# codex-storage/codex-storage-proofs-circuits

Measured on AMD Instinct MI355X. Metric: Poseidon2-BN254 permutations/sec per GPU; full proof-input witnesses/sec, higher is better.
Workload: dtype u32x9 (29-bit limbs, Montgomery mod BN254 r)

## Files before the change

### codex-storage-proofs-circuits_amd/csrc/internal.hpp

```cpp
#pragma once
#include <hip/hip_runtime.h>

#include <sys/resource.h>
#include <sys/syscall.h>
#include <unistd.h>

#include <condition_variable>
#include <cstdint>
#include <deque>
#include <functional>
#include <memory>
#include <mutex>
#include <string>
#include <thread>
#include <vector>

#include "../../include/codex_p2.h"
#include "workers.hpp"

namespace cp2i {

bool env_decimal(const char* name, uint64_t* value, bool* set);
bool env_keep_trees(int* mode);
size_t mem_limit_bytes();
hipError_t dev_malloc(void** p, size_t n);
void dev_free(void* p, size_t n);
size_t dev_bytes_held();
int device_free_bytes(size_t* out);

class BlockPool {
 public:
  static constexpr size_t MAX_CACHED_DEV = (size_t)6 << 30, MAX_CACHED_PIN = (size_t)4 << 30;
  ~BlockPool() { trim(); }
  void* get(bool pinned, size_t n, size_t* got) {
    if (n == 0) n = 16;
    {
      std::lock_guard<std::mutex> lk(mu_);
      auto& fl = pinned ? pin_ : dev_;
      size_t best = fl.size();
      for (size_t i = 0; i < fl.size(); ++i)
        if (fl[i].bytes >= n && fl[i].bytes / 4 <= n && (best == fl.size() || fl[i].bytes < fl[best].bytes)) best = i;
      if (best != fl.size()) {
        Blk b = fl[best];
        fl.erase(fl.begin() + (long)best);
        (pinned ? cached_pin_ : cached_dev_) -= b.bytes;
        *got = b.bytes;
        return b.p;
      }
    }
    size_t want = round_up(n);
    void* p = nullptr;
    hipError_t e = pinned ? hipHostMalloc(&p, want, hipHostMallocDefault) : dev_malloc(&p, want);
    if (e != hipSuccess) {
      (void)hipGetLastError();
      trim();
// ... 235 lines not shown
```

### codex-storage-proofs-circuits_amd/csrc/proof_many.cpp

```cpp
#include <hip/hip_runtime.h>

#include <algorithm>
#include <cstring>
#include <map>
#include <memory>
#include <string>
#include <vector>

#include "dataset_obj.hpp"
#include "proof_input_obj.hpp"
#include "trees.hpp"

using namespace cp2i;

namespace {

struct Req {
  cp2_dataset* ds = nullptr;
  uint64_t slot = 0;
  uint8_t entropy[32];
  size_t at = 0;
  size_t id = 0;
};

int refuse(cp2_ctx* ctx, size_t i, const std::string& why) {
  ctx->err = "request " + std::to_string(i) + ": " + why;
  return CP2_ERR_INVALID;
}

size_t depth_of(size_t n) { return layer_sizes_of(n).size() - 1; }

bool same_circuit(const cp2_config& a, const cp2_config& b) {
  return a.max_depth == b.max_depth && a.max_log2_nslots == b.max_log2_nslots && a.cell_size == b.cell_size && a.block_size == b.block_size &&
// ... 31 lines not shown
  CP2_TRY(d_a.scratch(ctx, n * 8));
  CP2_TRY(d_r.scratch(ctx, n * 32));
  CP2_HIP(ctx, hipMemcpyAsync(d_a.p, a.data(), n * 8, hipMemcpyHostToDevice, ctx->stream));
  CP2_HIP(ctx, cp2k::launch_gather_addr(static_cast<const uint64_t*>(d_a.p), n, 32, d_r.p, ctx->stream));
  CP2_HIP(ctx, hipMemcpyAsync(got.data(), d_r.p, n * 32, hipMemcpyDeviceToHost, ctx->stream));
  CP2_HIP(ctx, hipStreamSynchronize(ctx->stream));
  for (size_t i = 0; i < n; ++i)
    if (std::memcmp(&got[i * 32], &ds[i]->dlayers[slot_idx[i] * 32], 32) != 0)
      return refuse(ctx, i, "the root its dataset tree holds for slot " + std::to_string(slot_idx[i]) +
                                " (cp2_dataset_set_roots) differs from the slot's built root");
  return CP2_OK;
}

int prepare(cp2_ctx* ctx, cp2_dataset* const* ds, const uint64_t* slot_idx, size_t n) {
  CP2_TRY(validate(ctx, ds, slot_idx, n));
  CP2_HIP(ctx, hipSetDevice(ctx->device));
  for (size_t i = 0; i < n; ++i)
    if (!ds[i]->have_roots) CP2_TRY(cp2_dataset_set_roots(ds[i], nullptr));
  return check_roots(ctx, ds, slot_idx, n);
}

std::string who(bool named, const Req* r) { return named ? "request " + std::to_string(r->id) + ": " : std::string(); }

int run_pass(cp2_ctx* ctx, const std::vector<const Req*>& rq, size_t n_rf, size_t n_rfile, size_t n_cf, bool named, cp2_proof_input** out) {
  const size_t n = rq.size(), nr = n_rf + n_rfile;
  const cp2_config& c0 = rq[0]->ds->cfg;
  const size_t ns = c0.n_samples, md = (size_t)c0.max_depth, cs = c0.cell_size, bs = c0.block_size, cpb = bs / cs;
  const size_t T = n * ns, R = nr * ns, C = T - R, RF = n_rf * ns, CF = n_cf * ns;
  auto store = std::make_shared<BatchStore>();
  if (T) {
    std::vector<cp2k::ManyReq> reqs(n);
    std::vector<cp2k::TreeGeom> geoms;
    std::map<std::string, uint32_t> geom_of;
    for (size_t j = 0; j < n; ++j) {
      const cp2_dataset* ds = rq[j]->ds;
      cp2k::ManyReq& q = reqs[j];
      std::memset(&q, 0, sizeof q);
      std::memcpy(q.entropy, rq[j]->entropy, 32);
      std::memcpy(q.slot_root, &ds->dlayers[rq[j]->slot * 32], 32);
      q.n_cells = ds->cfg.n_cells;
      q.cpb = cpb;
      if (j < nr) {
        cp2k::TreeGeom g;
        std::memset(&g, 0, sizeof g);
        trees_geom(ds->trees, &g);
        auto it = geom_of.emplace(std::string(reinterpret_cast<const char*>(&g), sizeof g), (uint32_t)geoms.size());
        if (it.second) geoms.push_back(g);
        q.geom = it.first->second;
        q.nodes = (uint64_t)reinterpret_cast<uintptr_t>(ds->trees->nodes.p);
        q.slot = rq[j]->slot - ds->first_slot;
      }
    }
    std::vector<uint64_t> blk(C), gen, cpaths, ctail, ccell;
    std::vector<uint8_t> checks(2 * C * 32);
    PinBuf h_blocks;
    const size_t rows = T * md + T + 2 * C;
    DevBuf d_req, d_geom, d_idx, d_blk, d_addr, d_rows, d_cells, d_gen, d_caddr;
    CP2_TRY(d_req.scratch(ctx, n * sizeof(cp2k::ManyReq)));
    CP2_TRY(d_geom.scratch(ctx, std::max<size_t>(1, geoms.size()) * sizeof(cp2k::TreeGeom)));
    CP2_TRY(d_idx.scratch(ctx, T * 8));
    CP2_TRY(d_blk.scratch(ctx, T * 8));
    CP2_TRY(d_addr.scratch(ctx, rows * 8));
    CP2_TRY(d_rows.scratch(ctx, rows * 32));
    CP2_TRY(d_cells.scratch(ctx, (C * cpb + T) * cs));
    CP2_TRY(store->idx.alloc(ctx, T * 8));
    CP2_TRY(store->paths.alloc(ctx, T * md * 32));
    CP2_TRY(store->leaves.alloc(ctx, T * 32));
    CP2_TRY(store->cells.alloc(ctx, T * cs));
    uint8_t* cells_out = d_cells.u8() + C * cpb * cs;
    uint64_t* addr = static_cast<uint64_t*>(d_addr.p);
    CP2_HIP(ctx, hipMemcpyAsync(d_req.p, reqs.data(), n * sizeof(cp2k::ManyReq), hipMemcpyHostToDevice, ctx->stream));
    if (!geoms.empty())
      CP2_HIP(ctx, hipMemcpyAsync(d_geom.p, geoms.data(), geoms.size() * sizeof(cp2k::TreeGeom), hipMemcpyHostToDevice, ctx->stream));
    CP2_HIP(ctx, cp2k::launch_sample_many(static_cast<const cp2k::ManyReq*>(d_req.p), static_cast<const cp2k::TreeGeom*>(d_geom.p), n,
                                          (uint32_t)ns, (uint32_t)md, static_cast<uint64_t*>(d_idx.p), static_cast<uint64_t*>(d_blk.p), addr,
                                          ctx->stream));
    CP2_HIP(ctx, hipMemcpyAsync(store->idx.p, d_idx.p, T * 8, hipMemcpyDeviceToHost, ctx->stream));
    if (C) CP2_HIP(ctx, hipMemcpyAsync(blk.data(), static_cast<uint64_t*>(d_blk.p) + R, C * 8, hipMemcpyDeviceToHost, ctx->stream));
    CP2_HIP(ctx, hipStreamSynchronize(ctx->stream));
    const uint64_t* idx = static_cast<const uint64_t*>(store->idx.p);

    gen.assign((CF + RF) * 2, 0);
    uint64_t* seeds = gen.data();
    uint64_t* firsts = seeds + CF + RF;
    for (size_t q = 0; q < CF; ++q) {
      const Req* r = rq[nr + q / ns];
      seeds[q] = cp2_slot_seed(r->ds->cfg.seed, r->slot);
      firsts[q] = blk[q] * cpb;
    }
    for (size_t p = 0; p < RF; ++p) {
      const Req* r = rq[p / ns];
      seeds[CF + p] = cp2_slot_seed(r->ds->cfg.seed, r->slot);
      firsts[CF + p] = idx[p];
    }
    if (CF + RF) {
      CP2_TRY(d_gen.scratch(ctx, gen.size() * 8));
      const uint64_t* dg = static_cast<const uint64_t*>(d_gen.p);
      CP2_HIP(ctx, hipMemcpyAsync(d_gen.p, gen.data(), gen.size() * 8, hipMemcpyHostToDevice, ctx->stream));
      CP2_HIP(ctx, cp2k::launch_gen_fake_cells_many(dg, dg + CF + RF, cpb, CF * cpb, cs, d_cells.p, ctx->stream));
      CP2_HIP(ctx, cp2k::launch_gen_fake_cells_many(dg + CF, dg + CF + RF + CF, 1, RF, cs, cells_out, ctx->stream));
    }
    if (C > CF) {
      const size_t n_req_file = (C - CF) / ns;
      CP2_TRY(h_blocks.alloc(ctx, (C - CF) * bs));
      std::vector<std::string> failed(fill_threads(ctx));
      on_threads(fill_threads(ctx), n_req_file, [&](int w, size_t k) {
        const size_t q0 = CF + k * ns;
        const Req* r = rq[nr + q0 / ns];
        const std::string fname = slot_file_name(r->ds->file_base, r->slot);
        size_t bad = 0;
        const int err = slot_file_read_list(fname, ns, [&](size_t) { return bs; }, [&](size_t c) { return blk[q0 + c] * bs; },
                                            [&](size_t c) { return h_blocks.u8() + (q0 - CF + c) * bs; }, &bad);
        if (err >= 0)
          failed[w] = who(named, r) + (err ? "block " + std::to_string(blk[q0 + bad]) + " of slot " : std::string("slot ")) + std::to_string(r->slot) +
                      ": " + slot_file_error(fname, err);
        return err < 0;
      });
      for (const auto& f : failed)
        if (!f.empty()) { ctx->err = f; return CP2_ERR_IO; }
      CP2_HIP(ctx, hipMemcpyAsync(d_cells.u8() + CF * bs, h_blocks.p, (C - CF) * bs, hipMemcpyHostToDevice, ctx->stream));
    }
    cp2_slot_trees* mini = nullptr;
    struct Mini { cp2_slot_trees*& t; ~Mini() { cp2_slot_trees_free(t); } } mini_guard{mini};
    if (C) {
      cpaths.assign(C * md, 0);
      ctail.assign(3 * C, 0);
      ccell.assign(C, 0);
      CP2_TRY(cp2_slot_trees_build_dev(ctx, d_cells.p, C, cs, bs, cpb, &mini));
      const size_t depth_b = depth_of(cpb);
      const uint64_t mb = (uint64_t)reinterpret_cast<uintptr_t>(mini->nodes.p);
      std::vector<uint64_t> rr(depth_b + 1);
      for (size_t q = 0; q < C; ++q) {
        const Req* r = rq[nr + q / ns];
        const cp2_dataset* ds = r->ds;
        const uint64_t ls = r->slot - ds->first_slot, cell = idx[R + q], b = blk[q], in_block = cell % cpb;
        const uint64_t kb = (uint64_t)reinterpret_cast<uintptr_t>(ds->compact.p);
        uint64_t* P = &cpaths[q * md];
        path_rows(mini, q, in_block, depth_b + 1, rr.data());
        for (size_t d = 0; d < depth_b; ++d) P[d] = rr[d] == NO_ROW ? 0 : mb + rr[d] * 32;
        uint64_t j = b, m = ds->cfg.n_cells / cpb;
        for (size_t d = 0; d + 1 < ds->csizes.size(); ++d) {
          const uint64_t sib = j ^ 1;
          P[depth_b + d] = sib < m ? kb + (ds->coff[d] + ls * ds->csizes[d] + sib) * 32 : 0;
          j >>= 1;
          m = (m + 1) >> 1;
        }
        ctail[q] = mb + (q * cpb + in_block) * 32;
        ctail[C + 2 * q] = kb + (ds->coff[0] + ls * ds->csizes[0] + b) * 32;
        ctail[C + 2 * q + 1] = mb + (mini->toff[0] + q) * 32;
        ccell[q] = (uint64_t)reinterpret_cast<uintptr_t>(d_cells.u8()) + (q * cpb + in_block) * cs;
      }
      CP2_TRY(d_caddr.scratch(ctx, C * 8));
      CP2_HIP(ctx, hipMemcpyAsync(addr + R * md, cpaths.data(), C * md * 8, hipMemcpyHostToDevice, ctx->stream));
      CP2_HIP(ctx, hipMemcpyAsync(addr + T * md + R, ctail.data(), 3 * C * 8, hipMemcpyHostToDevice, ctx->stream));
      CP2_HIP(ctx, hipMemcpyAsync(d_caddr.p, ccell.data(), C * 8, hipMemcpyHostToDevice, ctx->stream));
      CP2_HIP(ctx, cp2k::launch_gather_addr(static_cast<const uint64_t*>(d_caddr.p), C, cs, cells_out + R * cs, ctx->stream));
    }
    CP2_HIP(ctx, cp2k::launch_gather_addr(addr, rows, 32, d_rows.p, ctx->stream));
    CP2_HIP(ctx, hipMemcpyAsync(store->paths.p, d_rows.p, T * md * 32, hipMemcpyDeviceToHost, ctx->stream));
    CP2_HIP(ctx, hipMemcpyAsync(store->leaves.p, d_rows.u8() + T * md * 32, T * 32, hipMemcpyDeviceToHost, ctx->stream));
    if (C) CP2_HIP(ctx, hipMemcpyAsync(checks.data(), d_rows.u8() + (T * md + T) * 32, 2 * C * 32, hipMemcpyDeviceToHost, ctx->stream));
    CP2_HIP(ctx, hipMemcpyAsync(store->cells.p, cells_out, T * cs, hipMemcpyDeviceToHost, ctx->stream));
    CP2_HIP(ctx, hipStreamSynchronize(ctx->stream));
    for (size_t q = 0; q < C; ++q)
      if (std::memcmp(&checks[2 * q * 32], &checks[(2 * q + 1) * 32], 32) != 0) {
        const Req* r = rq[nr + q / ns];
        ctx->err = who(named, r) + "block " + std::to_string(blk[q]) + " of slot " + std::to_string(r->slot) +
                   " does not hash to its stored root (slot data changed since the build?)";
        return CP2_ERR_IO;
      }
    if (R > RF) {
      std::vector<std::string> failed(fill_threads(ctx));
      on_threads(fill_threads(ctx), n_rfile, [&](int w, size_t k) {
        const Req* r = rq[n_rf + k];
        const std::string fname = slot_file_name(r->ds->file_base, r->slot);
        const size_t p0 = (n_rf + k) * ns;
        const int err = slot_file_read_list(fname, ns, [&](size_t) { return cs; }, [&](size_t c) { return idx[p0 + c] * cs; },
                                            [&](size_t c) { return store->cells.u8() + (p0 + c) * cs; });
        if (err >= 0) failed[w] = who(named, r) + slot_file_error(fname, err);
        return err < 0;
      });
      for (const auto& f : failed)
        if (!f.empty()) { ctx->err = f; return CP2_ERR_IO; }
    }
  }
  std::vector<ProofItem> items(n);
  for (size_t j = 0; j < n; ++j) items[j] = {rq[j]->ds, rq[j]->slot, rq[j]->entropy, &out[rq[j]->at]};
  return proof_inputs_from_store(items.data(), n, store, store->cells.u8());
}

}

int cp2i::prove_requests(cp2_ctx* ctx, cp2_dataset* const* ds, const uint64_t* slot_idx, const uint8_t* entropies, size_t n, size_t at0,
                         bool named, cp2_proof_input** out) {
  for (size_t i = 0; i < n; ++i) out[i] = nullptr;
  if (n == 0) return CP2_OK;
  CP2_HIP(ctx, hipSetDevice(ctx->device));
  std::vector<Req> req(n);
  std::vector<const Req*> res_fake, res_file, cmp_fake, cmp_file, roots_only;
  for (size_t i = 0; i < n; ++i) {
    req[i].ds = ds[i];
    req[i].slot = slot_idx[i];
    req[i].at = i;
    req[i].id = at0 + i;
    canonical_felt(entropies + 32 * i, req[i].entropy);
    const cp2_dataset* d = ds[i];
    (d->trees ? (d->from_file ? res_file : res_fake) : d->tree_mode == 2 ? (d->from_file ? cmp_file : cmp_fake) : roots_only).push_back(&req[i]);
  }
  auto fail = [&](int st) {
    for (size_t i = 0; i < n; ++i) { cp2_proof_input_free(out[i]); out[i] = nullptr; }
    return st;
  };
  for (const Req* r : roots_only) {
    const int st = cp2_proof_inputs_generate_batch(r->ds, &r->slot, 1, r->entropy, &out[r->at]);
    if (st != CP2_OK) {
      ctx->err = who(named, r) + ctx->err;
      return fail(st);
    }
  }
  const cp2_config& c0 = ds[0]->cfg;
  const size_t per_req = std::max<size_t>(1, (size_t)c0.n_samples * c0.block_size);
  const size_t chunk = std::max<size_t>(1, ctx->stage_bytes / per_req);
  std::vector<const Req*> compact(cmp_fake);
  compact.insert(compact.end(), cmp_file.begin(), cmp_file.end());
  const size_t n_res = res_fake.size() + res_file.size();
  size_t c = 0;
  for (bool first = true; first ? n_res + compact.size() > 0 : c < compact.size(); first = false) {
    std::vector<const Req*> rq;
    if (first) {
      rq = res_fake;
      rq.insert(rq.end(), res_file.begin(), res_file.end());
    }
    const size_t c1 = std::min(compact.size(), c + chunk);
    rq.insert(rq.end(), compact.begin() + (long)c, compact.begin() + (long)c1);
    const size_t n_cf = c < cmp_fake.size() ? std::min(c1, cmp_fake.size()) - c : 0;
    const int st = run_pass(ctx, rq, first ? res_fake.size() : 0, first ? res_file.size() : 0, n_cf, named, out);
    if (st != CP2_OK) return fail(st);
    c = c1;
  }
  return CP2_OK;
}

extern "C" int cp2_proof_inputs_generate_many(cp2_ctx* ctx, cp2_dataset* const* ds, const uint64_t* slot_idx, const uint8_t* entropies, size_t n,
                                              cp2_proof_input** out) try {
  if (!ctx) return CP2_ERR_INVALID;
  if (n && (!ds || !slot_idx || !entropies || !out)) {
    ctx->err = "cp2_proof_inputs_generate_many: NULL array";
    return CP2_ERR_INVALID;
  }
  for (size_t i = 0; i < n; ++i) out[i] = nullptr;
  if (n == 0) return CP2_OK;
  CP2_REFUSE_STUCK(ctx);
  CP2_TRY(prepare(ctx, ds, slot_idx, n));
  return prove_requests(ctx, ds, slot_idx, entropies, n, 0, true, out);
} catch (const std::bad_alloc&) {
  return CP2_ERR_ALLOC;
} catch (...) {
  return CP2_ERR_INVALID;
}

extern "C" int cp2_proof_inputs_export_many(cp2_ctx* ctx, cp2_dataset* const* ds, const uint64_t* slot_idx, const uint8_t* entropies, size_t n,
                                            const char* const* paths, int threads, size_t batch, uint64_t* total_bytes) try {
  if (!ctx) return CP2_ERR_INVALID;
// ... 17 lines not shown
```

### codex-storage-proofs-circuits_amd/csrc/slot_trees.cpp

```cpp
#include <hip/hip_runtime.h>

#include <fcntl.h>
#include <sys/mman.h>
#include <sys/stat.h>
#include <unistd.h>

#include <algorithm>
#include <atomic>
#include <chrono>
#include <cstdio>
#include <cstdlib>
#include <cstring>
#include <memory>
#include <new>
#include <string>
#include <vector>

#include "trees.hpp"
#include "fake_turns.hpp"
#include "ingest_turns.hpp"
#include "fill_pipeline.hpp"

using namespace cp2i;

// ... 270 lines not shown
  if (!ctx || !out || units_per_slot == 0) return CP2_ERR_INVALID;
  CP2_TRY(trees_check_geometry(cell_size, block_size, cells_per_unit, n_units));
  if (units_per_slot > 1 && !unit_geometry_ok(units_per_slot, cell_size, block_size, cells_per_unit)) return CP2_ERR_INVALID;
  return trees_build_fake(ctx, dataset_seed, first_unit, n_units, cell_size, block_size, cells_per_unit, 0, nullptr, out, units_per_slot);
} catch (const std::bad_alloc&) {
  return CP2_ERR_ALLOC;
} catch (...) {
  return CP2_ERR_INVALID;
}

extern "C" int cp2_slot_trees_build_file_units(cp2_ctx* ctx, const char* file_base, uint64_t units_per_slot, uint64_t first_unit,
                                               size_t n_units, size_t cell_size, size_t block_size, size_t cells_per_unit,
                                               cp2_slot_trees** out) try {
  if (!ctx || !out || !file_base || units_per_slot == 0 || cell_size > SLOT_FILE_MAX_CELL) return CP2_ERR_INVALID;
  CP2_TRY(trees_check_geometry(cell_size, block_size, cells_per_unit, n_units));
  if (units_per_slot > 1 && !unit_geometry_ok(units_per_slot, cell_size, block_size, cells_per_unit)) return CP2_ERR_INVALID;
  return trees_build_files(ctx, file_base, first_unit, n_units, cell_size, block_size, cells_per_unit, 0, nullptr, out, units_per_slot);
} catch (const std::bad_alloc&) {
  return CP2_ERR_ALLOC;
} catch (...) {
  return CP2_ERR_INVALID;
}

extern "C" int cp2_slot_trees_build_dev(cp2_ctx* ctx, const void* d_cells, size_t n_slots, size_t cell_size,
                                        size_t block_size, size_t n_cells, cp2_slot_trees** out) try {
  if (!ctx || !out || !d_cells) return CP2_ERR_INVALID;
  *out = nullptr;
  CP2_REFUSE_STUCK(ctx);
  CP2_TRY(trees_check_geometry(cell_size, block_size, n_cells, n_slots));
  CP2_HIP(ctx, hipSetDevice(ctx->device));
  std::unique_ptr<cp2_slot_trees> t(trees_new(ctx, n_slots, cell_size, block_size, n_cells));
  if (!t) return CP2_ERR_ALLOC;
  t->src = CellSrc::Dev;
  t->d_cells = static_cast<const uint8_t*>(d_cells);
  CP2_TRY(trees_layout(t.get()));
  CP2_HIP(ctx, cp2k::launch_hash_cells(d_cells, cell_size, n_slots * n_cells, t->nodes.p, ctx->stream));
  CP2_TRY(trees_build_layers(t.get(), 0, n_slots, ctx->stream));
  *out = t.release();
  return CP2_OK;
} catch (const std::bad_alloc&) {
  return CP2_ERR_ALLOC;
} catch (...) {
  return CP2_ERR_INVALID;
}

namespace {

size_t env_size(const char* name, size_t dflt) {
  const char* v = std::getenv(name);
  if (!v || !*v) return dflt;
  char* end = nullptr;
  unsigned long long x = std::strtoull(v, &end, 10);
  return (end && *end == 0 && x > 0) ? (size_t)x : dflt;
}

struct IngestPipe {
  static constexpr int MAX_DEPTH = 8;
  static constexpr size_t DIRECT_ALIGN = 4096;
  size_t cell_multiple = 1;
  cp2_ctx* ctx = nullptr;
  hipStream_t copy = nullptr;
  int pin_depth = 0, dev_depth = 0;
// ... 618 lines not shown
```

### codex-storage-proofs-circuits_amd/csrc/trees.hpp

```cpp
#pragma once
#include <functional>
#include <string>
#include <vector>

#include "batch_loop.hpp"
#include "internal.hpp"
#include "kernels.hpp"
#include "fill_pipeline.hpp"
#include "cache_file.hpp"

struct cp2_slot_trees {
  cp2_ctx* ctx = nullptr;
  size_t n_slots = 0, cell_size = 0, block_size = 0, n_cells = 0, cpb = 0, nblocks = 0;
  std::vector<size_t> bsizes, tsizes;
  std::vector<size_t> boff, toff;
  cp2i::DevBuf nodes;
  CellSrc src = CellSrc::Fake;
  uint64_t dataset_seed = 0, first_slot = 0;
  uint64_t units_per_slot = 1;
  bool pooled_nodes = false;
  const uint8_t* d_cells = nullptr;
  const uint8_t* h_cells = nullptr;
  std::string file_base;
};
// ... 20 lines not shown
int trees_build_fake(cp2_ctx* ctx, uint64_t dataset_seed, uint64_t first_slot, size_t n_slots, size_t cell_size, size_t block_size,
                     size_t n_cells, size_t group, const SlotsDone& done, cp2_slot_trees** out, uint64_t units_per_slot = 1,
                     bool pooled_nodes = false, BuildScratch* scratch = nullptr, int node_slot = 0);
int trees_build_files(cp2_ctx* ctx, const std::string& base, uint64_t first_slot, size_t n_slots, size_t cell_size,
                      size_t block_size, size_t n_cells, size_t group, const SlotsDone& done, cp2_slot_trees** out,
                      uint64_t units_per_slot = 1, bool pooled_nodes = false, BuildScratch* scratch = nullptr, int node_slot = 0);
int trees_build_file_list(cp2_ctx* ctx, const std::string* names, size_t n_names, size_t cell_size, size_t block_size, size_t n_cells,
                          size_t group, const SlotsDone& done, cp2_slot_trees** out, bool pooled_nodes = false,
                          BuildScratch* scratch = nullptr, int node_slot = 0);
struct ItemSource {
  bool from_file = false;
  std::string file_base;
  uint64_t seed = 0;
  size_t cell_size = 0, block_size = 0, n_cells = 0;
  uint64_t units_per_slot = 1;
  const std::string* names = nullptr;
  size_t n_names = 0;
};
ItemSource item_source_of(const cp2_slot_trees* t, uint64_t units_per_slot);
ItemSource item_source_of(const cp2_dataset* ds);
int build_items(cp2_ctx* ctx, const ItemSource& src, uint64_t s0, size_t n, size_t group, const SlotsDone& done, cp2_slot_trees** out,
                bool pooled_nodes = false, BuildScratch* scratch = nullptr, int node_slot = 0);

struct BatchDevice {
  using Tail = hipStream_t;
  cp2_ctx* ctx = nullptr;
  BuildScratch scratch;
  Event landed[2];
  cp2_slot_trees* batch = nullptr;
  ~BatchDevice() { release(); }
  int init(cp2_ctx* c) { ctx = c; CP2_TRY(landed[0].create(c)); return landed[1].create(c); }
  int wait(int b) { return cleared(hipEventSynchronize(landed[b]) == hipSuccess); }
  int record(int b, hipStream_t tail) {
    if (hipEventRecord(landed[b], tail) == hipSuccess) return CP2_OK;
    ctx->err = "hipEventRecord failed";
    return CP2_ERR_HIP;
  }
  int drain() {
    return cleared(hipStreamSynchronize(ctx->stream) == hipSuccess && (!ctx->aux_stream || hipStreamSynchronize(ctx->aux_stream) == hipSuccess) &&
                   (!ctx->aux2_stream || hipStreamSynchronize(ctx->aux2_stream) == hipSuccess));
  }
  void release() { cp2_slot_trees_free(batch); batch = nullptr; }
  int build(const ItemSource& src, uint64_t s0, size_t n, size_t group, const SlotsDone& done, int b, hipStream_t* tail) {
    const int st = build_items(ctx, src, s0, n, group, done, &batch, true, &scratch, b);
    *tail = scratch.tail_stream ? scratch.tail_stream : ctx->stream;
    return st;
// ... 35 lines not shown
```

Before: 731.6 million.

## Split proof-input generation into double-buffered passes overlapping host prep with device work

Restructures run_pass so compact-dataset requests are split into passes sized by stage_bytes. Each pass uses one of two preallocated pinned and device scratch sets and runs through a batch loop, so host block reads and address-table building for the next pass can overlap device gathering and hashing of the current one. Sampling for all requests now happens once up front, and mini-tree nodes go into a reusable buffer instead of a fresh allocation per call. The pinned cache cap is also raised. This adds pipeline and error-settling complexity and keeps two scratch sets resident, which costs more memory.

After: 731.6 million, median of 6. No clear change (-0.0%).

```diff
diff --git a/codex-storage-proofs-circuits_amd/csrc/internal.hpp b/codex-storage-proofs-circuits_amd/csrc/internal.hpp
--- a/codex-storage-proofs-circuits_amd/csrc/internal.hpp
+++ b/codex-storage-proofs-circuits_amd/csrc/internal.hpp
@@ -30,7 +30,7 @@
 
 class BlockPool {
  public:
-  static constexpr size_t MAX_CACHED_DEV = (size_t)6 << 30, MAX_CACHED_PIN = (size_t)4 << 30;
+  static constexpr size_t MAX_CACHED_DEV = (size_t)6 << 30, MAX_CACHED_PIN = (size_t)6 << 30;
   ~BlockPool() { trim(); }
   void* get(bool pinned, size_t n, size_t* got) {
     if (n == 0) n = 16;
diff --git a/codex-storage-proofs-circuits_amd/csrc/proof_many.cpp b/codex-storage-proofs-circuits_amd/csrc/proof_many.cpp
--- a/codex-storage-proofs-circuits_amd/csrc/proof_many.cpp
+++ b/codex-storage-proofs-circuits_amd/csrc/proof_many.cpp
@@ -9,6 +9,7 @@
 
 #include "dataset_obj.hpp"
 #include "proof_input_obj.hpp"
+#include "proof_pass_plan.hpp"
 #include "trees.hpp"
 
 using namespace cp2i;
@@ -86,25 +87,132 @@
 
 std::string who(bool named, const Req* r) { return named ? "request " + std::to_string(r->id) + ": " : std::string(); }
 
-int run_pass(cp2_ctx* ctx, const std::vector<const Req*>& rq, size_t n_rf, size_t n_rfile, size_t n_cf, bool named, cp2_proof_input** out) {
-  const size_t n = rq.size(), nr = n_rf + n_rfile;
-  const cp2_config& c0 = rq[0]->ds->cfg;
-  const size_t ns = c0.n_samples, md = (size_t)c0.max_depth, cs = c0.cell_size, bs = c0.block_size, cpb = bs / cs;
-  const size_t T = n * ns, R = nr * ns, C = T - R, RF = n_rf * ns, CF = n_cf * ns;
-  auto store = std::make_shared<BatchStore>();
-  if (T) {
-    std::vector<cp2k::ManyReq> reqs(n);
+struct Shape {
+  size_t n = 0, nr = 0, n_rf = 0, n_rfile = 0, n_cf = 0;
+  size_t T = 0, R = 0, C = 0, RF = 0, CF = 0;
+  size_t lane0 = 0;
+  size_t rows(size_t md) const { return T * md + T + 2 * C; }
+  size_t gen() const { return (CF + RF) * 2; }
+  size_t tab_words(size_t md) const { return gen() + C * md + 3 * C + C + 8 * C; }
+};
+
+struct PassSet {
+  DevBuf d_addr, d_rows, d_cells, d_gen, d_caddr, d_nodes;
+  PinBuf h_tab, h_blocks;
+  Shape s;
+  std::vector<const Req*> rq;
+  std::shared_ptr<BatchStore> store;
+  MiniGeom geom;
+  uint64_t* gen(size_t) const { return static_cast<uint64_t*>(h_tab.p); }
+  uint64_t* cpaths(size_t) const { return static_cast<uint64_t*>(h_tab.p) + s.gen(); }
+  uint64_t* ctail(size_t md) const { return cpaths(md) + s.C * md; }
+  uint64_t* ccell(size_t md) const { return ctail(md) + 3 * s.C; }
+  uint8_t* checks(size_t md) const { return reinterpret_cast<uint8_t*>(ccell(md) + s.C); }
+};
+
+struct PassDevice {
+  using Tail = hipStream_t;
+  cp2_ctx* ctx = nullptr;
+  PassSet set[2];
+  Event landed[2], uploaded[2];
+  cp2_slot_trees* mini = nullptr;
+  ~PassDevice() {
+    release();
+    if (ctx && !ctx->stuck) (void)drain();
+  }
+  int init(cp2_ctx* c) {
+    ctx = c;
+    for (int b = 0; b < 2; ++b) { CP2_TRY(landed[b].create(c)); CP2_TRY(uploaded[b].create(c)); }
+    return CP2_OK;
+  }
+  int wait(int b) { return BatchDevice::cleared(hipEventSynchronize(landed[b]) == hipSuccess); }
+  int record(int b, hipStream_t tail) {
+    if (hipEventRecord(landed[b], tail) == hipSuccess) return CP2_OK;
+    ctx->err = "hipEventRecord failed";
+    return CP2_ERR_HIP;
+  }
+  int drain() {
+    return BatchDevice::cleared(hipStreamSynchronize(ctx->stream) == hipSuccess && (!ctx->aux_stream || hipStreamSynchronize(ctx->aux_stream) == hipSuccess) &&
+                                (!ctx->aux2_stream || hipStreamSynchronize(ctx->aux2_stream) == hipSuccess));
+  }
+  void release() { cp2_slot_trees_free(mini); mini = nullptr; }
+};
+
+struct Call {
+  cp2_ctx* ctx = nullptr;
+  bool named = false;
+  cp2_proof_input** out = nullptr;
+  size_t ns = 0, md = 0, cs = 0, bs = 0, cpb = 0;
+  std::vector<const Req*> res, compact;
+  size_t n_rf = 0, n_cmp_fake = 0;
+  PassCut cut;
+  PinBuf h_idx, h_blk;
+  const uint64_t* idx() const { return static_cast<const uint64_t*>(h_idx.p); }
+  const uint64_t* blk() const { return static_cast<const uint64_t*>(h_blk.p); }
+
+  Shape shape(size_t k) const {
+    const PassSlice sl = pass_slice(cut, compact.size(), k);
+    Shape s;
+    s.nr = k ? 0 : res.size();
+    s.n_rf = k ? 0 : n_rf;
+    s.n_rfile = s.nr - s.n_rf;
+    s.n_cf = sl.c0 < n_cmp_fake ? std::min(sl.c1, n_cmp_fake) - sl.c0 : 0;
+    s.n = s.nr + (sl.c1 - sl.c0);
+    s.T = s.n * ns, s.R = s.nr * ns, s.C = s.T - s.R, s.RF = s.n_rf * ns, s.CF = s.n_cf * ns;
+    s.lane0 = k ? res.size() * ns + sl.c0 * ns : 0;
+    return s;
+  }
+  std::vector<const Req*> requests(size_t k) const {
+    const PassSlice sl = pass_slice(cut, compact.size(), k);
+    std::vector<const Req*> rq;
+    if (k == 0) rq = res;
+    rq.insert(rq.end(), compact.begin() + (long)sl.c0, compact.begin() + (long)sl.c1);
+    return rq;
+  }
+
+  int alloc_sets(PassDevice& dev) const {
+    for (int b = 0; b < 2; ++b) {
+      Shape m;
+      size_t nodes = 0, file_lanes = 0, tab = 0;
+      for (size_t k = (size_t)b; k < cut.passes; k += 2) {
+        const Shape s = shape(k);
+        m.T = std::max(m.T, s.T), m.C = std::max(m.C, s.C);
+        m.CF = std::max(m.CF, s.CF), m.RF = std::max(m.RF, s.RF);
+        nodes = std::max<size_t>(nodes, mini_geom(s.C, cpb).rows * 32);
+        file_lanes = std::max(file_lanes, s.C - s.CF);
+        tab = std::max(tab, s.tab_words(md));
+      }
+      if (m.T == 0) continue;
+      PassSet& S = dev.set[b];
+      CP2_TRY(S.d_addr.scratch(ctx, m.rows(md) * 8));
+      CP2_TRY(S.d_rows.scratch(ctx, m.rows(md) * 32));
+      CP2_TRY(S.d_cells.scratch(ctx, (m.C * cpb + m.T) * cs));
+      if (m.gen()) CP2_TRY(S.d_gen.scratch(ctx, m.gen() * 8));
+      if (m.C) CP2_TRY(S.d_caddr.scratch(ctx, m.C * 8));
+      if (m.C) CP2_TRY(S.d_nodes.scratch(ctx, nodes));
+      CP2_TRY(S.h_tab.alloc(ctx, tab * 8));
+      if (file_lanes) CP2_TRY(S.h_blocks.alloc(ctx, file_lanes * bs));
+    }
+    return CP2_OK;
+  }
+
+  int sample(PassDevice& dev) {
+    const size_t n_all = res.size() + compact.size(), T_all = n_all * ns;
+    const Shape s0 = shape(0);
+    const size_t n_first = res.empty() ? n_all : s0.n;
+    std::vector<cp2k::ManyReq> reqs(n_all);
     std::vector<cp2k::TreeGeom> geoms;
     std::map<std::string, uint32_t> geom_of;
-    for (size_t j = 0; j < n; ++j) {
-      const cp2_dataset* ds = rq[j]->ds;
+    for (size_t j = 0; j < n_all; ++j) {
+      const Req* r = j < res.size() ? res[j] : compact[j - res.size()];
+      const cp2_dataset* ds = r->ds;
       cp2k::ManyReq& q = reqs[j];
       std::memset(&q, 0, sizeof q);
-      std::memcpy(q.entropy, rq[j]->entropy, 32);
-      std::memcpy(q.slot_root, &ds->dlayers[rq[j]->slot * 32], 32);
+      std::memcpy(q.entropy, r->entropy, 32);
+      std::memcpy(q.slot_root, &ds->dlayers[r->slot * 32], 32);
       q.n_cells = ds->cfg.n_cells;
       q.cpb = cpb;
-      if (j < nr) {
+      if (j < res.size()) {
         cp2k::TreeGeom g;
         std::memset(&g, 0, sizeof g);
         trees_geom(ds->trees, &g);
@@ -112,146 +220,187 @@
         if (it.second) geoms.push_back(g);
         q.geom = it.first->second;
         q.nodes = (uint64_t)reinterpret_cast<uintptr_t>(ds->trees->nodes.p);
-        q.slot = rq[j]->slot - ds->first_slot;
-      }
-    }
-    std::vector<uint64_t> blk(C), gen, cpaths, ctail, ccell;
-    std::vector<uint8_t> checks(2 * C * 32);
-    PinBuf h_blocks;
-    const size_t rows = T * md + T + 2 * C;
-    DevBuf d_req, d_geom, d_idx, d_blk, d_addr, d_rows, d_cells, d_gen, d_caddr;
-    CP2_TRY(d_req.scratch(ctx, n * sizeof(cp2k::ManyReq)));
+        q.slot = r->slot - ds->first_slot;
+      }
+    }
+    DevBuf d_req, d_geom, d_idx, d_blk;
+    CP2_TRY(d_req.scratch(ctx, n_all * sizeof(cp2k::ManyReq)));
     CP2_TRY(d_geom.scratch(ctx, std::max<size_t>(1, geoms.size()) * sizeof(cp2k::TreeGeom)));
-    CP2_TRY(d_idx.scratch(ctx, T * 8));
-    CP2_TRY(d_blk.scratch(ctx, T * 8));
-    CP2_TRY(d_addr.scratch(ctx, rows * 8));
-    CP2_TRY(d_rows.scratch(ctx, rows * 32));
-    CP2_TRY(d_cells.scratch(ctx, (C * cpb + T) * cs));
-    CP2_TRY(store->idx.alloc(ctx, T * 8));
-    CP2_TRY(store->paths.alloc(ctx, T * md * 32));
-    CP2_TRY(store->leaves.alloc(ctx, T * 32));
-    CP2_TRY(store->cells.alloc(ctx, T * cs));
-    uint8_t* cells_out = d_cells.u8() + C * cpb * cs;
-    uint64_t* addr = static_cast<uint64_t*>(d_addr.p);
-    CP2_HIP(ctx, hipMemcpyAsync(d_req.p, reqs.data(), n * sizeof(cp2k::ManyReq), hipMemcpyHostToDevice, ctx->stream));
+    CP2_TRY(d_idx.scratch(ctx, T_all * 8));
+    CP2_TRY(d_blk.scratch(ctx, T_all * 8));
+    CP2_TRY(h_idx.alloc(ctx, T_all * 8));
+    CP2_TRY(h_blk.alloc(ctx, T_all * 8));
+    const cp2k::ManyReq* dq = static_cast<const cp2k::ManyReq*>(d_req.p);
+    const cp2k::TreeGeom* dg = static_cast<const cp2k::TreeGeom*>(d_geom.p);
+    uint64_t* di = static_cast<uint64_t*>(d_idx.p);
+    uint64_t* db = static_cast<uint64_t*>(d_blk.p);
+    uint64_t* addr0 = static_cast<uint64_t*>(dev.set[0].d_addr.p);
+    CP2_HIP(ctx, hipMemcpyAsync(d_req.p, reqs.data(), n_all * sizeof(cp2k::ManyReq), hipMemcpyHostToDevice, ctx->stream));
     if (!geoms.empty())
       CP2_HIP(ctx, hipMemcpyAsync(d_geom.p, geoms.data(), geoms.size() * sizeof(cp2k::TreeGeom), hipMemcpyHostToDevice, ctx->stream));
-    CP2_HIP(ctx, cp2k::launch_sample_many(static_cast<const cp2k::ManyReq*>(d_req.p), static_cast<const cp2k::TreeGeom*>(d_geom.p), n,
-                                          (uint32_t)ns, (uint32_t)md, static_cast<uint64_t*>(d_idx.p), static_cast<uint64_t*>(d_blk.p), addr,
-                                          ctx->stream));
-    CP2_HIP(ctx, hipMemcpyAsync(store->idx.p, d_idx.p, T * 8, hipMemcpyDeviceToHost, ctx->stream));
-    if (C) CP2_HIP(ctx, hipMemcpyAsync(blk.data(), static_cast<uint64_t*>(d_blk.p) + R, C * 8, hipMemcpyDeviceToHost, ctx->stream));
+    CP2_HIP(ctx, cp2k::launch_sample_many(dq, dg, n_first, (uint32_t)ns, (uint32_t)md, di, db, addr0, ctx->stream));
+    if (n_all > n_first)
+      CP2_HIP(ctx, cp2k::launch_sample_many(dq + n_first, dg, n_all - n_first, (uint32_t)ns, (uint32_t)md, di + n_first * ns, db + n_first * ns, addr0,
+                                            ctx->stream));
+    CP2_HIP(ctx, hipMemcpyAsync(h_idx.p, d_idx.p, T_all * 8, hipMemcpyDeviceToHost, ctx->stream));
+    CP2_HIP(ctx, hipMemcpyAsync(h_blk.p, d_blk.p, T_all * 8, hipMemcpyDeviceToHost, ctx->stream));
     CP2_HIP(ctx, hipStreamSynchronize(ctx->stream));
-    const uint64_t* idx = static_cast<const uint64_t*>(store->idx.p);
-
-    gen.assign((CF + RF) * 2, 0);
-    uint64_t* seeds = gen.data();
-    uint64_t* firsts = seeds + CF + RF;
-    for (size_t q = 0; q < CF; ++q) {
-      const Req* r = rq[nr + q / ns];
+    return CP2_OK;
+  }
+
+  int prepare(PassDevice& dev, size_t k, int b) const {
+    PassSet& S = dev.set[b];
+    S.s = shape(k);
+    S.rq = requests(k);
+    const Shape& s = S.s;
+    S.store = std::make_shared<BatchStore>();
+    CP2_TRY(S.store->idx.alloc(ctx, s.T * 8));
+    CP2_TRY(S.store->paths.alloc(ctx, s.T * md * 32));
+    CP2_TRY(S.store->leaves.alloc(ctx, s.T * 32));
+    CP2_TRY(S.store->cells.alloc(ctx, s.T * cs));
+    const uint64_t* pidx = idx() + s.lane0;
+    const uint64_t* pblk = blk() + s.lane0 + s.R;
+    std::memcpy(S.store->idx.p, pidx, s.T * 8);
+    uint64_t* seeds = S.gen(md);
+    uint64_t* firsts = seeds + s.CF + s.RF;
+    for (size_t q = 0; q < s.CF; ++q) {
+      const Req* r = S.rq[s.nr + q / ns];
       seeds[q] = cp2_slot_seed(r->ds->cfg.seed, r->slot);
-      firsts[q] = blk[q] * cpb;
-    }
-    for (size_t p = 0; p < RF; ++p) {
-      const Req* r = rq[p / ns];
-      seeds[CF + p] = cp2_slot_seed(r->ds->cfg.seed, r->slot);
-      firsts[CF + p] = idx[p];
-    }
-    if (CF + RF) {
-      CP2_TRY(d_gen.scratch(ctx, gen.size() * 8));
-      const uint64_t* dg = static_cast<const uint64_t*>(d_gen.p);
-      CP2_HIP(ctx, hipMemcpyAsync(d_gen.p, gen.data(), gen.size() * 8, hipMemcpyHostToDevice, ctx->stream));
-      CP2_HIP(ctx, cp2k::launch_gen_fake_cells_many(dg, dg + CF + RF, cpb, CF * cpb, cs, d_cells.p, ctx->stream));
-      CP2_HIP(ctx, cp2k::launch_gen_fake_cells_many(dg + CF, dg + CF + RF + CF, 1, RF, cs, cells_out, ctx->stream));
-    }
-    if (C > CF) {
-      const size_t n_req_file = (C - CF) / ns;
-      CP2_TRY(h_blocks.alloc(ctx, (C - CF) * bs));
+      firsts[q] = pblk[q] * cpb;
+    }
+    for (size_t p = 0; p < s.RF; ++p) {
+      const Req* r = S.rq[p / ns];
+      seeds[s.CF + p] = cp2_slot_seed(r->ds->cfg.seed, r->slot);
+      firsts[s.CF + p] = pidx[p];
+    }
+    if (s.C > s.CF) {
+      const size_t n_req_file = (s.C - s.CF) / ns;
+      if (!S.h_blocks.p || S.h_blocks.bytes < (s.C - s.CF) * bs) {
+        ctx->err = "proof passes: no landing zone for a pass's blocks";
+        return CP2_ERR_INVALID;
+      }
       std::vector<std::string> failed(fill_threads(ctx));
-      on_threads(fill_threads(ctx), n_req_file, [&](int w, size_t k) {
-        const size_t q0 = CF + k * ns;
-        const Req* r = rq[nr + q0 / ns];
+      on_threads(fill_threads(ctx), n_req_file, [&](int w, size_t f) {
+        const size_t q0 = s.CF + f * ns;
+        const Req* r = S.rq[s.nr + q0 / ns];
         const std::string fname = slot_file_name(r->ds->file_base, r->slot);
         size_t bad = 0;
-        const int err = slot_file_read_list(fname, ns, [&](size_t) { return bs; }, [&](size_t c) { return blk[q0 + c] * bs; },
-                                            [&](size_t c) { return h_blocks.u8() + (q0 - CF + c) * bs; }, &bad);
+        const int err = slot_file_read_list(fname, ns, [&](size_t) { return bs; }, [&](size_t c) { return pblk[q0 + c] * bs; },
+                                            [&](size_t c) { return S.h_blocks.u8() + (q0 - s.CF + c) * bs; }, &bad);
         if (err >= 0)
-          failed[w] = who(named, r) + (err ? "block " + std::to_string(blk[q0 + bad]) + " of slot " : std::string("slot ")) + std::to_string(r->slot) +
+          failed[w] = who(named, r) + (err ? "block " + std::to_string(pblk[q0 + bad]) + " of slot " : std::string("slot ")) + std::to_string(r->slot) +
                       ": " + slot_file_error(fname, err);
         return err < 0;
       });
       for (const auto& f : failed)
         if (!f.empty()) { ctx->err = f; return CP2_ERR_IO; }
-      CP2_HIP(ctx, hipMemcpyAsync(d_cells.u8() + CF * bs, h_blocks.p, (C - CF) * bs, hipMemcpyHostToDevice, ctx->stream));
-    }
-    cp2_slot_trees* mini = nullptr;
-    struct Mini { cp2_slot_trees*& t; ~Mini() { cp2_slot_trees_free(t); } } mini_guard{mini};
-    if (C) {
-      cpaths.assign(C * md, 0);
-      ctail.assign(3 * C, 0);
-      ccell.assign(C, 0);
-      CP2_TRY(cp2_slot_trees_build_dev(ctx, d_cells.p, C, cs, bs, cpb, &mini));
-      const size_t depth_b = depth_of(cpb);
-      const uint64_t mb = (uint64_t)reinterpret_cast<uintptr_t>(mini->nodes.p);
-      std::vector<uint64_t> rr(depth_b + 1);
-      for (size_t q = 0; q < C; ++q) {
-        const Req* r = rq[nr + q / ns];
+    }
+    S.geom = mini_geom(s.C, cpb);
+    if (s.C) {
+      if (S.d_nodes.bytes < S.geom.rows * 32 || S.d_cells.bytes < (s.C * cpb + s.T) * cs) {
+        ctx->err = "proof passes: a scratch set smaller than its pass";
+        return CP2_ERR_INVALID;
+      }
+      const uint64_t mb = (uint64_t)reinterpret_cast<uintptr_t>(S.d_nodes.p), cb = (uint64_t)reinterpret_cast<uintptr_t>(S.d_cells.p);
+      uint64_t* cpaths = S.cpaths(md);
+      uint64_t* ctail = S.ctail(md);
+      uint64_t* ccell = S.ccell(md);
+      for (size_t q = 0; q < s.C; ++q) {
+        const Req* r = S.rq[s.nr + q / ns];
         const cp2_dataset* ds = r->ds;
-        const uint64_t ls = r->slot - ds->first_slot, cell = idx[R + q], b = blk[q], in_block = cell % cpb;
-        const uint64_t kb = (uint64_t)reinterpret_cast<uintptr_t>(ds->compact.p);
-        uint64_t* P = &cpaths[q * md];
-        path_rows(mini, q, in_block, depth_b + 1, rr.data());
-        for (size_t d = 0; d < depth_b; ++d) P[d] = rr[d] == NO_ROW ? 0 : mb + rr[d] * 32;
-        uint64_t j = b, m = ds->cfg.n_cells / cpb;
-        for (size_t d = 0; d + 1 < ds->csizes.size(); ++d) {
-          const uint64_t sib = j ^ 1;
-          P[depth_b + d] = sib < m ? kb + (ds->coff[d] + ls * ds->csizes[d] + sib) * 32 : 0;
-          j >>= 1;
-          m = (m + 1) >> 1;
-        }
-        ctail[q] = mb + (q * cpb + in_block) * 32;
-        ctail[C + 2 * q] = kb + (ds->coff[0] + ls * ds->csizes[0] + b) * 32;
-        ctail[C + 2 * q + 1] = mb + (mini->toff[0] + q) * 32;
-        ccell[q] = (uint64_t)reinterpret_cast<uintptr_t>(d_cells.u8()) + (q * cpb + in_block) * cs;
-      }
-      CP2_TRY(d_caddr.scratch(ctx, C * 8));
-      CP2_HIP(ctx, hipMemcpyAsync(addr + R * md, cpaths.data(), C * md * 8, hipMemcpyHostToDevice, ctx->stream));
-      CP2_HIP(ctx, hipMemcpyAsync(addr + T * md + R, ctail.data(), 3 * C * 8, hipMemcpyHostToDevice, ctx->stream));
-      CP2_HIP(ctx, hipMemcpyAsync(d_caddr.p, ccell.data(), C * 8, hipMemcpyHostToDevice, ctx->stream));
-      CP2_HIP(ctx, cp2k::launch_gather_addr(static_cast<const uint64_t*>(d_caddr.p), C, cs, cells_out + R * cs, ctx->stream));
-    }
-    CP2_HIP(ctx, cp2k::launch_gather_addr(addr, rows, 32, d_rows.p, ctx->stream));
-    CP2_HIP(ctx, hipMemcpyAsync(store->paths.p, d_rows.p, T * md * 32, hipMemcpyDeviceToHost, ctx->stream));
-    CP2_HIP(ctx, hipMemcpyAsync(store->leaves.p, d_rows.u8() + T * md * 32, T * 32, hipMemcpyDeviceToHost, ctx->stream));
-    if (C) CP2_HIP(ctx, hipMemcpyAsync(checks.data(), d_rows.u8() + (T * md + T) * 32, 2 * C * 32, hipMemcpyDeviceToHost, ctx->stream));
-    CP2_HIP(ctx, hipMemcpyAsync(store->cells.p, cells_out, T * cs, hipMemcpyDeviceToHost, ctx->stream));
-    CP2_HIP(ctx, hipStreamSynchronize(ctx->stream));
-    for (size_t q = 0; q < C; ++q)
+        const KeptTree kept{(uint64_t)reinterpret_cast<uintptr_t>(ds->compact.p), r->slot - ds->first_slot, ds->cfg.n_cells / cpb,
+                            ds->csizes.data(), ds->coff.data(), ds->csizes.size()};
+        const LaneAddr a = pass_lane_addresses(S.geom, mb, cb, cs, q, pidx[s.R + q], pblk[q], kept, md, &cpaths[q * md]);
+        ctail[q] = a.leaf;
+        ctail[s.C + 2 * q] = a.stored_root;
+        ctail[s.C + 2 * q + 1] = a.rebuilt_root;
+        ccell[q] = a.cell;
+      }
+    }
+    return CP2_OK;
+  }
+
+  int enqueue(PassDevice& dev, int b, hipStream_t* tail) const {
+    PassSet& S = dev.set[b];
+    const Shape& s = S.s;
+    hipStream_t st = ctx->stream;
+    *tail = st;
+    uint64_t* addr = static_cast<uint64_t*>(S.d_addr.p);
+    uint8_t* cells_out = S.d_cells.u8() + s.C * cpb * cs;
+    if (s.CF + s.RF) {
+      const uint64_t* dg = static_cast<const uint64_t*>(S.d_gen.p);
+      CP2_HIP(ctx, hipMemcpyAsync(S.d_gen.p, S.gen(md), s.gen() * 8, hipMemcpyHostToDevice, st));
+      CP2_HIP(ctx, cp2k::launch_gen_fake_cells_many(dg, dg + s.CF + s.RF, cpb, s.CF * cpb, cs, S.d_cells.p, st));
+      CP2_HIP(ctx, cp2k::launch_gen_fake_cells_many(dg + s.CF, dg + s.CF + s.RF + s.CF, 1, s.RF, cs, cells_out, st));
+    }
+    if (s.C > s.CF) {
+      hipStream_t up = nullptr;
+      CP2_TRY(aux_stream(ctx, &up));
+      CP2_HIP(ctx, hipStreamWaitEvent(up, dev.landed[b], 0));
+      CP2_HIP(ctx, hipMemcpyAsync(S.d_cells.u8() + s.CF * bs, S.h_blocks.p, (s.C - s.CF) * bs, hipMemcpyHostToDevice, up));
+      CP2_HIP(ctx, hipEventRecord(dev.uploaded[b], up));
+      CP2_HIP(ctx, hipStreamWaitEvent(st, dev.uploaded[b], 0));
+    }
+    if (s.C) {
+      CP2_TRY(trees_build_dev_into(ctx, S.d_cells.p, s.C, cs, bs, cpb, &S.d_nodes, &dev.mini));
+      const cp2_slot_trees* t = dev.mini;
+      bool same = t->nodes.p == S.d_nodes.p && t->bsizes.size() == S.geom.bsz.size() && t->toff[0] == S.geom.roots && t->nodes.bytes == S.geom.rows * 32;
+      for (size_t l = 0; same && l < t->bsizes.size(); ++l) same = t->bsizes[l] == S.geom.bsz[l] && t->boff[l] == S.geom.boff[l];
+      if (!same) {
+        ctx->err = "proof passes: the rebuilt blocks are not laid out as planned";
+        return CP2_ERR_INVALID;
+      }
+      CP2_HIP(ctx, hipMemcpyAsync(addr + s.R * md, S.cpaths(md), s.C * md * 8, hipMemcpyHostToDevice, st));
+      CP2_HIP(ctx, hipMemcpyAsync(addr + s.T * md + s.R, S.ctail(md), 3 * s.C * 8, hipMemcpyHostToDevice, st));
+      CP2_HIP(ctx, hipMemcpyAsync(S.d_caddr.p, S.ccell(md), s.C * 8, hipMemcpyHostToDevice, st));
+      CP2_HIP(ctx, cp2k::launch_gather_addr(static_cast<const uint64_t*>(S.d_caddr.p), s.C, cs, cells_out + s.R * cs, st));
+    }
+    CP2_HIP(ctx, cp2k::launch_gather_addr(addr, s.rows(md), 32, S.d_rows.p, st));
+    CP2_HIP(ctx, hipMemcpyAsync(S.store->paths.p, S.d_rows.p, s.T * md * 32, hipMemcpyDeviceToHost, st));
+    CP2_HIP(ctx, hipMemcpyAsync(S.store->leaves.p, S.d_rows.u8() + s.T * md * 32, s.T * 32, hipMemcpyDeviceToHost, st));
+    if (s.C) CP2_HIP(ctx, hipMemcpyAsync(S.checks(md), S.d_rows.u8() + (s.T * md + s.T) * 32, 2 * s.C * 32, hipMemcpyDeviceToHost, st));
+    CP2_HIP(ctx, hipMemcpyAsync(S.store->cells.p, cells_out, s.T * cs, hipMemcpyDeviceToHost, st));
+    return CP2_OK;
+  }
+
+  int finish(PassDevice& dev, size_t k) const {
+    PassSet& S = dev.set[k & 1];
+    const Shape& s = S.s;
+    if (dev.wait((int)(k & 1)) != CP2_OK) {
+      ctx->err = "proof inputs: a pass failed on the device";
+      return CP2_ERR_HIP;
+    }
+    const uint8_t* checks = S.checks(md);
+    const uint64_t* pidx = idx() + s.lane0;
+    const uint64_t* pblk = blk() + s.lane0 + s.R;
+    for (size_t q = 0; q < s.C; ++q)
       if (std::memcmp(&checks[2 * q * 32], &checks[(2 * q + 1) * 32], 32) != 0) {
-        const Req* r = rq[nr + q / ns];
-        ctx->err = who(named, r) + "block " + std::to_string(blk[q]) + " of slot " + std::to_string(r->slot) +
+        const Req* r = S.rq[s.nr + q / ns];
+        ctx->err = who(named, r) + "block " + std::to_string(pblk[q]) + " of slot " + std::to_string(r->slot) +
                    " does not hash to its stored root (slot data changed since the build?)";
         return CP2_ERR_IO;
       }
-    if (R > RF) {
+    if (s.R > s.RF) {
       std::vector<std::string> failed(fill_threads(ctx));
-      on_threads(fill_threads(ctx), n_rfile, [&](int w, size_t k) {
-        const Req* r = rq[n_rf + k];
+      on_threads(fill_threads(ctx), s.n_rfile, [&](int w, size_t f) {
+        const Req* r = S.rq[s.n_rf + f];
         const std::string fname = slot_file_name(r->ds->file_base, r->slot);
-        const size_t p0 = (n_rf + k) * ns;
-        const int err = slot_file_read_list(fname, ns, [&](size_t) { return cs; }, [&](size_t c) { return idx[p0 + c] * cs; },
-                                            [&](size_t c) { return store->cells.u8() + (p0 + c) * cs; });
+        const size_t p0 = (s.n_rf + f) * ns;
+        const int err = slot_file_read_list(fname, ns, [&](size_t) { return cs; }, [&](size_t c) { return pidx[p0 + c] * cs; },
+                                            [&](size_t c) { return S.store->cells.u8() + (p0 + c) * cs; });
         if (err >= 0) failed[w] = who(named, r) + slot_file_error(fname, err);
         return err < 0;
       });
       for (const auto& f : failed)
         if (!f.empty()) { ctx->err = f; return CP2_ERR_IO; }
     }
-  }
-  std::vector<ProofItem> items(n);
-  for (size_t j = 0; j < n; ++j) items[j] = {rq[j]->ds, rq[j]->slot, rq[j]->entropy, &out[rq[j]->at]};
-  return proof_inputs_from_store(items.data(), n, store, store->cells.u8());
-}
+    std::vector<ProofItem> items(s.n);
+    for (size_t j = 0; j < s.n; ++j) items[j] = {S.rq[j]->ds, S.rq[j]->slot, S.rq[j]->entropy, &out[S.rq[j]->at]};
+    const std::shared_ptr<BatchStore> store = std::move(S.store);
+    S.store.reset();
+    return proof_inputs_from_store(items.data(), s.n, store, store->cells.u8());
+  }
+};
 
 }
 
@@ -283,26 +432,39 @@
     }
   }
   const cp2_config& c0 = ds[0]->cfg;
-  const size_t per_req = std::max<size_t>(1, (size_t)c0.n_samples * c0.block_size);
-  const size_t chunk = std::max<size_t>(1, ctx->stage_bytes / per_req);
-  std::vector<const Req*> compact(cmp_fake);
-  compact.insert(compact.end(), cmp_file.begin(), cmp_file.end());
-  const size_t n_res = res_fake.size() + res_file.size();
-  size_t c = 0;
-  for (bool first = true; first ? n_res + compact.size() > 0 : c < compact.size(); first = false) {
-    std::vector<const Req*> rq;
-    if (first) {
-      rq = res_fake;
-      rq.insert(rq.end(), res_file.begin(), res_file.end());
-    }
-    const size_t c1 = std::min(compact.size(), c + chunk);
-    rq.insert(rq.end(), compact.begin() + (long)c, compact.begin() + (long)c1);
-    const size_t n_cf = c < cmp_fake.size() ? std::min(c1, cmp_fake.size()) - c : 0;
-    const int st = run_pass(ctx, rq, first ? res_fake.size() : 0, first ? res_file.size() : 0, n_cf, named, out);
-    if (st != CP2_OK) return fail(st);
-    c = c1;
-  }
-  return CP2_OK;
+  Call call;
+  call.ctx = ctx;
+  call.named = named;
+  call.out = out;
+  call.ns = c0.n_samples, call.md = (size_t)c0.max_depth, call.cs = c0.cell_size, call.bs = c0.block_size, call.cpb = call.bs / call.cs;
+  call.res = res_fake;
+  call.res.insert(call.res.end(), res_file.begin(), res_file.end());
+  call.n_rf = res_fake.size();
+  call.compact = cmp_fake;
+  call.compact.insert(call.compact.end(), cmp_file.begin(), cmp_file.end());
+  call.n_cmp_fake = cmp_fake.size();
+  const size_t per_req = std::max<size_t>(1, call.ns * call.bs);
+  call.cut = pass_cut(call.compact.size(), std::max<size_t>(1, ctx->stage_bytes / per_req), !call.res.empty());
+  if (call.cut.passes == 0) return CP2_OK;
+  if (call.ns == 0) {
+    std::vector<const Req*> rq = call.res;
+    rq.insert(rq.end(), call.compact.begin(), call.compact.end());
+    std::vector<ProofItem> items(rq.size());
+    for (size_t j = 0; j < rq.size(); ++j) items[j] = {rq[j]->ds, rq[j]->slot, rq[j]->entropy, &out[rq[j]->at]};
+    auto store = std::make_shared<BatchStore>();
+    const int st = proof_inputs_from_store(items.data(), items.size(), store, store->cells.u8());
+    return st == CP2_OK ? st : fail(st);
+  }
+  PassDevice dev;
+  int st = dev.init(ctx);
+  if (st == CP2_OK) st = call.alloc_sets(dev);
+  if (st == CP2_OK) st = call.sample(dev);
+  if (st == CP2_OK)
+    st = pass_loop(dev, "proof inputs", ctx->err, call.cut.passes,
+                   [&](const BatchStep& s) { return call.prepare(dev, s.k, s.b); },
+                   [&](const BatchStep& s, hipStream_t* tail) { return call.enqueue(dev, s.b, tail); },
+                   [&](size_t k) { return call.finish(dev, k); });
+  return st == CP2_OK ? st : fail(st);
 }
 
 extern "C" int cp2_proof_inputs_generate_many(cp2_ctx* ctx, cp2_dataset* const* ds, const uint64_t* slot_idx, const uint8_t* entropies, size_t n,
diff --git a/codex-storage-proofs-circuits_amd/csrc/proof_pass_plan.hpp b/codex-storage-proofs-circuits_amd/csrc/proof_pass_plan.hpp
--- /dev/null
+++ b/codex-storage-proofs-circuits_amd/csrc/proof_pass_plan.hpp
@@ -0,0 +1,117 @@
+#pragma once
+#include <algorithm>
+#include <cstddef>
+#include <cstdint>
+#include <string>
+#include <vector>
+
+#include "batch_loop.hpp"
+
+namespace cp2i {
+
+struct PassCut { size_t passes = 0, per = 0; };
+inline PassCut pass_cut(size_t m, size_t cap, bool resident) {
+  PassCut c;
+  cap = std::max<size_t>(1, cap);
+  c.passes = m / cap + (m % cap != 0);
+  c.per = c.passes ? m / c.passes + (m % c.passes != 0) : 0;
+  if (!c.passes && resident) c.passes = 1;
+  return c;
+}
+struct PassSlice { size_t c0 = 0, c1 = 0; };
+inline PassSlice pass_slice(const PassCut& c, size_t m, size_t k) {
+  PassSlice s;
+  s.c0 = std::min(m, k * c.per);
+  s.c1 = std::min(m, s.c0 + c.per);
+  return s;
+}
+
+inline std::vector<uint64_t> pass_layer_sizes(uint64_t n) {
+  std::vector<uint64_t> s;
+  if (n == 0) return s;
+  bool bottom = true;
+  for (uint64_t m = n;; m = (m + 1) / 2, bottom = false) {
+    s.push_back(m);
+    if (m == 1 && !bottom) break;
+  }
+  return s;
+}
+struct MiniGeom {
+  uint64_t lanes = 0, cpb = 0;
+  std::vector<uint64_t> bsz, boff;
+  uint64_t roots = 0;
+  uint64_t rows = 0;
+  size_t depth() const { return bsz.empty() ? 0 : bsz.size() - 1; }
+};
+inline MiniGeom mini_geom(uint64_t lanes, uint64_t cpb) {
+  MiniGeom g;
+  g.lanes = lanes;
+  g.cpb = cpb;
+  g.bsz = pass_layer_sizes(cpb);
+  uint64_t off = 0;
+  for (size_t k = 0; k < g.bsz.size(); ++k) {
+    g.boff.push_back(off);
+    if (k + 1 < g.bsz.size()) off += lanes * g.bsz[k];
+  }
+  g.roots = off;
+  g.rows = off + 2 * lanes;
+  return g;
+}
+
+struct KeptTree {
+  uint64_t base = 0;
+  uint64_t local_slot = 0;
+  uint64_t n_blocks = 0;
+  const size_t* csizes = nullptr;
+  const size_t* coff = nullptr;
+  size_t n_layers = 0;
+};
+struct LaneAddr { uint64_t leaf = 0, stored_root = 0, rebuilt_root = 0, cell = 0; };
+inline LaneAddr pass_lane_addresses(const MiniGeom& g, uint64_t mini_base, uint64_t cells_base, uint64_t cell_size, uint64_t q, uint64_t cell,
+                                    uint64_t blk, const KeptTree& t, size_t md, uint64_t* P) {
+  const uint64_t in_block = cell % g.cpb;
+  const size_t depth_b = g.depth();
+  for (size_t d = 0; d < md; ++d) P[d] = 0;
+  uint64_t j = in_block, m = g.cpb;
+  for (size_t d = 0; d < depth_b && d < md; ++d) {
+    const uint64_t sib = j ^ 1;
+    if (sib < m) P[d] = mini_base + (g.boff[d] + q * g.bsz[d] + sib) * 32;
+    j >>= 1;
+    m = (m + 1) >> 1;
+  }
+  j = blk;
+  m = t.n_blocks;
+  for (size_t d = 0; d + 1 < t.n_layers && depth_b + d < md; ++d) {
+    const uint64_t sib = j ^ 1;
+    if (sib < m) P[depth_b + d] = t.base + (t.coff[d] + t.local_slot * t.csizes[d] + sib) * 32;
+    j >>= 1;
+    m = (m + 1) >> 1;
+  }
+  LaneAddr a;
+  a.leaf = mini_base + (q * g.cpb + in_block) * 32;
+  a.stored_root = t.base + (t.coff[0] + t.local_slot * t.csizes[0] + blk) * 32;
+  a.rebuilt_root = mini_base + (g.roots + q) * 32;
+  a.cell = cells_base + (q * g.cpb + in_block) * cell_size;
+  return a;
+}
+
+template <typename Device, typename Prepare, typename Enqueue, typename Finish>
+int pass_loop(Device& dev, const char* what, std::string& err, size_t n_passes, Prepare prepare, Enqueue enqueue, Finish finish) {
+  const auto settle = [&](const BatchStep& s, int st) {
+    if (s.k == 0) return st;
+    const std::string text = err;
+    const int before = finish(s.k - 1);
+    if (before != CP2_OK) return before;
+    err = text;
+    return st;
+  };
+  const int st = batch_loop(dev, what, err, n_passes, 1,
+      [&](const BatchStep& s) { const int p = prepare(s); return p == CP2_OK ? p : settle(s, p); },
+      [&](const BatchStep& s, typename Device::Tail* tail) { const int e = enqueue(s, tail); return e == CP2_OK ? e : settle(s, e); },
+      [&](const BatchStep& s, typename Device::Tail) { return s.k ? finish(s.k - 1) : CP2_OK; },
+      [](const BatchStep&) {});
+  if (st != CP2_OK || n_passes == 0) return st;
+  return finish(n_passes - 1);
+}
+
+}
diff --git a/codex-storage-proofs-circuits_amd/csrc/slot_trees.cpp b/codex-storage-proofs-circuits_amd/csrc/slot_trees.cpp
--- a/codex-storage-proofs-circuits_amd/csrc/slot_trees.cpp
+++ b/codex-storage-proofs-circuits_amd/csrc/slot_trees.cpp
@@ -316,22 +316,31 @@
   return CP2_ERR_INVALID;
 }
 
-extern "C" int cp2_slot_trees_build_dev(cp2_ctx* ctx, const void* d_cells, size_t n_slots, size_t cell_size,
-                                        size_t block_size, size_t n_cells, cp2_slot_trees** out) try {
-  if (!ctx || !out || !d_cells) return CP2_ERR_INVALID;
+int cp2i::trees_build_dev_into(cp2_ctx* ctx, const void* d_cells, size_t n_slots, size_t cell_size, size_t block_size, size_t n_cells,
+                               DevBuf* nodes, cp2_slot_trees** out) {
   *out = nullptr;
   CP2_REFUSE_STUCK(ctx);
   CP2_TRY(trees_check_geometry(cell_size, block_size, n_cells, n_slots));
+  if (nodes && (!nodes->p || nodes->bytes < trees_node_bytes(n_slots, cell_size, block_size, n_cells))) {
+    ctx->err = "device builder: the node buffer it was given is too small";
+    return CP2_ERR_INVALID;
+  }
   CP2_HIP(ctx, hipSetDevice(ctx->device));
   std::unique_ptr<cp2_slot_trees> t(trees_new(ctx, n_slots, cell_size, block_size, n_cells));
   if (!t) return CP2_ERR_ALLOC;
   t->src = CellSrc::Dev;
   t->d_cells = static_cast<const uint8_t*>(d_cells);
-  CP2_TRY(trees_layout(t.get()));
+  CP2_TRY(trees_layout(t.get(), nodes));
   CP2_HIP(ctx, cp2k::launch_hash_cells(d_cells, cell_size, n_slots * n_cells, t->nodes.p, ctx->stream));
   CP2_TRY(trees_build_layers(t.get(), 0, n_slots, ctx->stream));
   *out = t.release();
   return CP2_OK;
+}
+
+extern "C" int cp2_slot_trees_build_dev(cp2_ctx* ctx, const void* d_cells, size_t n_slots, size_t cell_size,
+                                        size_t block_size, size_t n_cells, cp2_slot_trees** out) try {
+  if (!ctx || !out || !d_cells) return CP2_ERR_INVALID;
+  return trees_build_dev_into(ctx, d_cells, n_slots, cell_size, block_size, n_cells, nullptr, out);
 } catch (const std::bad_alloc&) {
   return CP2_ERR_ALLOC;
 } catch (...) {
diff --git a/codex-storage-proofs-circuits_amd/csrc/trees.hpp b/codex-storage-proofs-circuits_amd/csrc/trees.hpp
--- a/codex-storage-proofs-circuits_amd/csrc/trees.hpp
+++ b/codex-storage-proofs-circuits_amd/csrc/trees.hpp
@@ -66,6 +66,9 @@
 int build_items(cp2_ctx* ctx, const ItemSource& src, uint64_t s0, size_t n, size_t group, const SlotsDone& done, cp2_slot_trees** out,
                 bool pooled_nodes = false, BuildScratch* scratch = nullptr, int node_slot = 0);
 
+int trees_build_dev_into(cp2_ctx* ctx, const void* d_cells, size_t n_slots, size_t cell_size, size_t block_size, size_t n_cells, DevBuf* nodes,
+                         cp2_slot_trees** out);
+
 struct BatchDevice {
   using Tail = hipStream_t;
   cp2_ctx* ctx = nullptr;
```
